# diver-j/melgan-multi

Hardware: NVIDIA H100
Metric: generator_fwd_audio_frames_per_sec (higher is better)
Workload: dtype f32 in/out; products as 3 split-bf16 wgmma passes with fp32 accumulation (fp32-equivalent, ~1e-5)

## Files before the change

melgan_multi_b200/csrc/mg_api.cu:

```cuda
#include <new>
#include <stdlib.h>
#include <string.h>

#include "mg_common.cuh"

namespace mg {


static int *status_ptr(void *workspace, int B, int T) {
    return reinterpret_cast<int *>(reinterpret_cast<float *>(workspace) + ws_offset(6, (size_t)B, (size_t)T));
}

static int run_generator(const float *packed, const float *mel, float *audio, const RunTable &batch, float *ws, cudaStream_t s,
                         cudaEvent_t *ev, const float *mel_host = nullptr, float *audio_host = nullptr) {
    int *st = status_ptr(ws, batch.items(), batch.stride);
    MG_CUDA_TRY(cudaMemsetAsync(st, 0, sizeof(int), s));
    return launch_generator_tc(packed, mel, audio, batch, ws, st, s, ev, mel_host, audio_host);
}

static int check_shape(const char *fn, int B, int T) {
    if (B < 1 || T < 1) return set_error(MG_ERR_INVALID_ARGUMENT, "%s: need B >= 1 and T >= 1 (got B=%d, T=%d)", fn, B, T);
    if ((long long)B * T > (1ll << 24)) return set_error(MG_ERR_INVALID_ARGUMENT, "%s: B*T = %lld too large", fn, (long long)B * T);
    return MG_OK;
}
// ... 126 lines not shown
    int rc = check_shape("mg_gen_stage_output", B, T);
    if (rc) return rc;
    if (which < 0 || which > 3 || !workspace || !out)
        return set_error(MG_ERR_INVALID_ARGUMENT, "mg_gen_stage_output: which must be 0..3 (the last stage is fused with conv_post)");
    if (which > 0 && generator_tc_tail() != 0)
        return set_error(MG_ERR_INVALID_ARGUMENT, "mg_gen_stage_output: ResBlock outputs are not materialised while the next stage's "
                         "ConvT is fused at their kernel's tail; select the unfused chain with mg_gen_set_pipeline(0) first");
    const size_t off = ws_offset(which, B, T), n = ws_offset(which + 1, B, T) - off;
    MG_CUDA_TRY(cudaMemcpyAsync(out, (const float *)workspace + off, n * sizeof(float), cudaMemcpyDeviceToDevice,
                                (cudaStream_t)stream));
    return MG_OK;
}

size_t mg_msd_grouped_backward_workspace_bytes(int layer, int Bt, int Lout) {
    if (layer < 1 || layer > 4 || Bt < 1 || Lout < 1) return 0;
    return grouped_bwd_workspace_bytes(layer, Bt, Lout);
}

int mg_msd_grouped_backward(const void *packed, int scale, int layer, const float *dz, const float *x, float *dx, float *dw,
                            float *db, void *workspace, size_t workspace_bytes, int Bt, int Lin, int Lout, void *stream) {
    if (!packed || !dz || scale < 0 || scale > 2 || layer < 1 || layer > 4 || Bt < 1 || Lin < 1 || Lout < 1)
        return set_error(MG_ERR_INVALID_ARGUMENT, "mg_msd_grouped_backward: bad argument");
    const DLayer d = d_layer(layer);
    if (Lout != (Lin + 2 * d.pad - d.k) / d.stride + 1)
        return set_error(MG_ERR_INVALID_ARGUMENT, "mg_msd_grouped_backward: Lout %d does not follow from Lin %d", Lout, Lin);
    if (dw && (!x || !db || !workspace || workspace_bytes < grouped_bwd_workspace_bytes(layer, Bt, Lout)))
        return set_error(MG_ERR_WORKSPACE_TOO_SMALL, "mg_msd_grouped_backward: dw needs x, db and a workspace of %zu bytes",
                         grouped_bwd_workspace_bytes(layer, Bt, Lout));
    const uint8_t *blob = reinterpret_cast<const uint8_t *>(packed) + (size_t)scale * d_blob_bytes();
    return launch_disc_grouped_backward(blob, layer, dz, x, dx, dw, db, (float *)workspace, Bt, Lin, Lout, (cudaStream_t)stream);
}

int mg_msd_post1_dgrad(const void *packed, int scale, const float *dz, float *dx, int Bt, int L, void *status_word, void *stream) {
    if (!packed || !dz || !dx || dz == dx || !status_word || scale < 0 || scale > 2 || Bt < 1 || L < 1)
        return set_error(MG_ERR_INVALID_ARGUMENT, "mg_msd_post1_dgrad: bad argument");
    const uint8_t *blob = reinterpret_cast<const uint8_t *>(packed) + (size_t)scale * d_blob_bytes();
    return launch_disc_post1_dgrad_tc(dz, dx, blob + d_tcT_start(), reinterpret_cast<const float *>(blob + d_zero_start()), Bt, L,
                                      (int *)status_word, (cudaStream_t)stream);
}

int mg_msd_post1_wgrad(const float *x, const float *dz, float *dw, float *db, int Bt, int L, void *status_word, void *stream) {
    if (!x || !dz || !dw || !db || !status_word || Bt < 1 || L < 1)
        return set_error(MG_ERR_INVALID_ARGUMENT, "mg_msd_post1_wgrad: bad argument");
    return launch_disc_post1_wgrad_tc(x, dz, dw, db, Bt, L, (int *)status_word, (cudaStream_t)stream);
}

size_t mg_msd_edge_backward_workspace_bytes(int layer, int Bt, int L) {
    return (layer == 0 && Bt > 0 && L > 0) ? edge_bwd_workspace_bytes(layer, Bt, L) : 0;
}

int mg_msd_edge_backward(const void *packed, int scale, int layer, const float *dz, const float *x, float *dx, float *dw, float *db,
                         void *workspace, size_t workspace_bytes, int Bt, int L, void *stream) {
    if (!packed || !dz || !x || !dw || !db || scale < 0 || scale > 2 || (layer != 0 && layer != 6) || Bt < 1 || L < 1)
        return set_error(MG_ERR_INVALID_ARGUMENT, "mg_msd_edge_backward: bad argument (layer is 0 = conv_pre or 6 = conv_post2)");
    if (layer == 0 && (!workspace || workspace_bytes < edge_bwd_workspace_bytes(0, Bt, L)))
        return set_error(MG_ERR_WORKSPACE_TOO_SMALL, "mg_msd_edge_backward: conv_pre needs a workspace of %zu bytes",
                         edge_bwd_workspace_bytes(0, Bt, L));
    const uint8_t *blob = reinterpret_cast<const uint8_t *>(packed) + (size_t)scale * d_blob_bytes();
    return launch_disc_edge_backward(blob, layer, dz, x, dx, dw, db, (float *)workspace, Bt, L, (cudaStream_t)stream);
}

size_t mg_msd_scale_backward_workspace_bytes(int Bt, int L0) {
    return (Bt > 0 && L0 > 0) ? disc_scale_backward_workspace_bytes(Bt, L0) : 0;
}

int mg_msd_scale_backward(const void *packed, int scale, const float *x0, const float *const *fmap, const float *const *gfmap,
                          float *gx0, float *const *dw, float *const *db, int *reached, void *workspace, size_t workspace_bytes,
                          int Bt, int L0, void *status_word, void *stream) {
    if (!packed || !x0 || !fmap || !gfmap || !dw || !db || !workspace || !status_word || scale < 0 || scale > 2 || Bt < 1 || L0 < 1)
        return set_error(MG_ERR_INVALID_ARGUMENT, "mg_msd_scale_backward: bad argument");
    for (int l = 0; l < kDiscLayers; ++l)
        if (!fmap[l]) return set_error(MG_ERR_INVALID_ARGUMENT, "mg_msd_scale_backward: fmap[%d] is NULL", l);
    if (Bt > 65535) return set_error(MG_ERR_INVALID_ARGUMENT, "discriminator batch %d exceeds 65535", Bt);
    const uint8_t *blob = reinterpret_cast<const uint8_t *>(packed) + (size_t)scale * d_blob_bytes();
    return launch_disc_scale_backward(blob, x0, fmap, gfmap, gx0, dw, db, reached, workspace, workspace_bytes, Bt, L0,
                                      (int *)status_word, (cudaStream_t)stream);
}

int mg_lrelu_backward(const float *g1, const float *g2, const float *out, float *dz, long long n, void *stream) {
    return launch_lrelu_grad(g1, g2, out, dz, n, (cudaStream_t)stream);
}

int mg_msd_wn_backward(const float *const *v, const float *const *g, const float *const *dw, float *const *dv,
                       float *const *dg, void *stream) {
    if (!v || !g || !dw || !dv || !dg) return set_error(MG_ERR_INVALID_ARGUMENT, "mg_msd_wn_backward: null argument");
    return launch_disc_wn_backward(v, g, dw, dv, dg, (cudaStream_t)stream);
}

int mg_adam_chunk(void) { return 4096; }

int mg_adam_step(float *const *p, const float *const *g, float *const *m, float *const *v, const long long *n,
                 const int *first, int count, int total_ctas, float lr, float beta1, float beta2, float eps,
                 float weight_decay, long long step, void *stream) {
    return launch_adam(p, g, m, v, n, first, count, total_ctas, lr, beta1, beta2, eps, weight_decay, step, (cudaStream_t)stream);
}

size_t mg_loss_workspace_bytes(const long long *n, int count) {
    if (!n || count < 1) return 0;
    return (size_t)loss_num_ctas(n, count) * sizeof(float);
}

int mg_loss_forward(const float *const *a, const float *const *b, const long long *n, const int *mode, int count,
                    float *out, void *workspace, size_t workspace_bytes, void *stream) {
    if (!out || !workspace) return set_error(MG_ERR_INVALID_ARGUMENT, "mg_loss_forward: null argument");
    if (n && count >= 1 && workspace_bytes < mg_loss_workspace_bytes(n, count))
        return set_error(MG_ERR_WORKSPACE_TOO_SMALL, "mg_loss_forward: workspace too small");
    return launch_loss_forward(a, b, n, mode, count, out, (float *)workspace, (cudaStream_t)stream);
}

int mg_loss_backward(const float *const *a, const float *const *b, const long long *n, const int *mode, int count,
                     const float *grad_out, float *const *grad_a, float *const *grad_b, void *stream) {
    if (!grad_out) return set_error(MG_ERR_INVALID_ARGUMENT, "mg_loss_backward: null grad_out");
    return launch_loss_backward(a, b, n, mode, count, grad_out, grad_a, grad_b, (cudaStream_t)stream);
}

int mg_gen_forward_launches(void) { return generator_tc_num_launches(); }

int mg_gen_forward_slices(int B, int T) { return (B >= 1 && T >= 1) ? generator_tc_slices(B, (long long)B * T) : 1; }

int mg_gen_check_status(const void *workspace, int B, int T, void *stream) {
    int rc = check_shape("mg_gen_check_status", B, T);
    if (rc) return rc;
    if (!workspace) return set_error(MG_ERR_INVALID_ARGUMENT, "mg_gen_check_status: null workspace");
    MG_CUDA_TRY(cudaStreamSynchronize((cudaStream_t)stream));
    int st = 0;
    MG_CUDA_TRY(cudaMemcpy(&st, status_ptr(const_cast<void *>(workspace), B, T), sizeof(int), cudaMemcpyDeviceToHost));
    if (st) return set_error(MG_ERR_CUDA, "tensor-core pipeline wait timed out (role code %d)", st);
    return MG_OK;
}

int mg_gen_convt(const void *packed, int stage, const float *x, float *y, int B, int Lin, void *stream) {
    if (!packed || !x || !y || x == y || stage < 0 || stage > 3 || B < 1 || Lin < 1)
        return set_error(MG_ERR_INVALID_ARGUMENT, "mg_gen_convt: bad argument");
    return run_one_kernel("mg_gen_convt", (cudaStream_t)stream, [&](int *st) {
        return launch_convt_tc(x, y, (const float *)packed, stage, RunTable::uniform(B, Lin), st, (cudaStream_t)stream);
    });
}

int mg_gen_conv_pre(const void *packed, const float *mel, float *y, int B, int T, void *stream) {
    if (!packed || !mel || !y || B < 1 || T < 1) return set_error(MG_ERR_INVALID_ARGUMENT, "mg_gen_conv_pre: bad argument");
    return run_one_kernel("mg_gen_conv_pre", (cudaStream_t)stream, [&](int *st) {
        return launch_gen_pre_tc(mel, y, (const float *)packed, RunTable::uniform(B, T), st, (cudaStream_t)stream);
    });
}

int mg_gen_resblock_post(const void *packed, const float *x, float *audio, int B, int L, void *stream) {
    if (!packed || !x || !audio || B < 1 || L < 1) return set_error(MG_ERR_INVALID_ARGUMENT, "mg_gen_resblock_post: bad argument");
    return run_one_kernel("mg_gen_resblock_post", (cudaStream_t)stream, [&](int *st) {
        return launch_resblock_tc(x, audio, (const float *)packed, 4, RunTable::uniform(B, L), st, (cudaStream_t)stream);
    });
}

int mg_gen_resblock_trace(const void *packed, int stage, const float *x, float *y, int B, int L, long long *trace_host) {
    if (!packed || !x || !y || x == y || !trace_host || stage < 0 || stage > 3)
        return set_error(MG_ERR_INVALID_ARGUMENT, "mg_gen_resblock_trace: bad argument");
    int *st = nullptr;
    long long *tr = nullptr;
    MG_CUDA_TRY(cudaMalloc(&st, sizeof(int)));
    MG_CUDA_TRY(cudaMalloc(&tr, 128 * sizeof(long long)));
    cudaMemset(st, 0, sizeof(int));
    cudaMemset(tr, 0, 128 * sizeof(long long));
    int rc = launch_resblock_tc(x, y, (const float *)packed, stage, RunTable::uniform(B, L), st, 0, tr);
    if (rc == MG_OK && cudaDeviceSynchronize() != cudaSuccess) rc = set_error(MG_ERR_CUDA, "mg_gen_resblock_trace: kernel failed");
    if (rc == MG_OK) cudaMemcpy(trace_host, tr, 128 * sizeof(long long), cudaMemcpyDeviceToHost);
    cudaFree(st);
    cudaFree(tr);
    return rc;
}

int mg_gen_resblock(const void *packed, int stage, const float *x, float *y, int B, int L, void *stream) {
    if (!packed || !x || !y || x == y || stage < 0 || stage > 3 || B < 1 || L < 1)
        return set_error(MG_ERR_INVALID_ARGUMENT, "mg_gen_resblock: bad argument");
    return run_one_kernel("mg_gen_resblock", (cudaStream_t)stream, [&](int *st) {
        return launch_resblock_tc(x, y, (const float *)packed, stage, RunTable::uniform(B, L), st, (cudaStream_t)stream);
    });
}

int mg_gen_resup(const void *packed, int stage, const float *x, float *y, int B, int L, void *stream) {
    if (!packed || !x || !y || x == y || stage < 0 || stage > 2 || B < 1 || L < 1)
        return set_error(MG_ERR_INVALID_ARGUMENT, "mg_gen_resup: bad argument");
    return run_one_kernel("mg_gen_resup", (cudaStream_t)stream, [&](int *st) {
        return launch_resblock_tc(x, y, (const float *)packed, 20 + stage, RunTable::uniform(B, L), st, (cudaStream_t)stream);
    });
}

int mg_gen_upres(const void *packed, int stage, const float *x, float *y, int B, int Lin, void *stream) {
    if (!packed || !x || !y || x == y || (stage != 2 && stage != 3) || B < 1 || Lin < 1)
        return set_error(MG_ERR_INVALID_ARGUMENT, "mg_gen_upres: bad argument");
    return run_one_kernel("mg_gen_upres", (cudaStream_t)stream, [&](int *st) {
        return launch_resblock_tc(x, y, (const float *)packed, 10 + stage, RunTable::uniform(B, 2 * Lin), st, (cudaStream_t)stream);
    });
}

int mg_gen_upres_post(const void *packed, const float *x, float *audio, int B, int Lin, void *stream) {
    if (!packed || !x || !audio || (const void *)x == (const void *)audio || B < 1 || Lin < 1)
        return set_error(MG_ERR_INVALID_ARGUMENT, "mg_gen_upres_post: bad argument");
    return run_one_kernel("mg_gen_upres_post", (cudaStream_t)stream, [&](int *st) {
        return launch_resblock_tc(x, audio, (const float *)packed, 14, RunTable::uniform(B, 2 * Lin), st, (cudaStream_t)stream);
    });
}

const char *mg_gen_resblock_config(int code) { return resblock_config_name(code, 0); }


size_t mg_msd_packed_bytes(void) { return msd_packed_bytes(); }

int mg_msd_pack(const float *const *v, const float *const *g, const float *const *bias, void *packed, void *stream) {
    if (!v || !g || !bias || !packed) return set_error(MG_ERR_INVALID_ARGUMENT, "mg_msd_pack: null argument");
    if ((uintptr_t)packed % 256) return set_error(MG_ERR_INVALID_ARGUMENT, "mg_msd_pack: packed must be 256-byte aligned");
    return launch_disc_pack(v, g, bias, packed, (cudaStream_t)stream);
}

int mg_msd_lengths(int L, int *lens) {
    if (L < 1 || !lens) return set_error(MG_ERR_INVALID_ARGUMENT, "mg_msd_lengths: bad argument");
    msd_lengths(L, lens);
    for (int i = 0; i < 21; ++i)
        if (lens[i] < 1) return set_error(MG_ERR_INVALID_ARGUMENT, "mg_msd_lengths: L = %d is too short for the discriminators", L);
    return MG_OK;
}

int mg_msd_forward(const void *packed, const float *y, int Bt, int L, float *const *fmaps, void *status_word, void *stream) {
    if (!packed || !y || !fmaps || !status_word || Bt < 1 || L < 1)
        return set_error(MG_ERR_INVALID_ARGUMENT, "mg_msd_forward: bad argument");
    int lens[21];
    int rc = mg_msd_lengths(L, lens);
    if (rc) return rc;
    for (int i = 0; i < 21; ++i)
        if (!fmaps[i]) return set_error(MG_ERR_INVALID_ARGUMENT, "mg_msd_forward: null feature-map pointer %d", i);
    MG_CUDA_TRY(cudaMemsetAsync(status_word, 0, sizeof(int), (cudaStream_t)stream));
    return launch_msd_forward(packed, y, Bt, L, fmaps, (int *)status_word, (cudaStream_t)stream);
}

size_t mg_disc_packed_bytes(void) { return d_blob_bytes(); }

int mg_disc_pack(const float *const *v, const float *const *g, const float *const *bias, void *packed, void *stream) {
    if (!v || !g || !bias || !packed) return set_error(MG_ERR_INVALID_ARGUMENT, "mg_disc_pack: null argument");
    if ((uintptr_t)packed % 256) return set_error(MG_ERR_INVALID_ARGUMENT, "mg_disc_pack: packed must be 256-byte aligned");
    return launch_disc_pack(v, g, bias, packed, (cudaStream_t)stream, 1);
}

int mg_disc_forward(const void *packed, const float *x, int Bt, int L, float *const *fmaps, void *status_word, void *stream) {
    if (!packed || !x || !fmaps || !status_word || Bt < 1 || L < 1)
        return set_error(MG_ERR_INVALID_ARGUMENT, "mg_disc_forward: bad argument");
    int lens[21];
    msd_lengths(L, lens);
    for (int i = 0; i < 7; ++i) {
        if (lens[i] < 1) return set_error(MG_ERR_INVALID_ARGUMENT, "mg_disc_forward: L = %d is too short", L);
        if (!fmaps[i]) return set_error(MG_ERR_INVALID_ARGUMENT, "mg_disc_forward: null feature-map pointer %d", i);
    }
    MG_CUDA_TRY(cudaMemsetAsync(status_word, 0, sizeof(int), (cudaStream_t)stream));
    return launch_disc_forward(packed, x, Bt, L, fmaps, (int *)status_word, (cudaStream_t)stream);
}

int mg_msd_check_status(const void *status_word, void *stream) {
    if (!status_word) return set_error(MG_ERR_INVALID_ARGUMENT, "mg_msd_check_status: null argument");
    MG_CUDA_TRY(cudaStreamSynchronize((cudaStream_t)stream));
    int st = 0;
    MG_CUDA_TRY(cudaMemcpy(&st, status_word, sizeof(int), cudaMemcpyDeviceToHost));
    if (st) return set_error(MG_ERR_CUDA, "tensor-core pipeline wait timed out (role code %d)", st);
    return MG_OK;
}


size_t mg_mel_tables_bytes(void) { return mel_tables_bytes(); }

int mg_mel_tables_build(int sampling_rate, int n_mels, float fmin, float fmax, int norm, void *tables_host) {
    if (!tables_host) return set_error(MG_ERR_INVALID_ARGUMENT, "mg_mel_tables_build: null buffer");
    return mel_tables_build(sampling_rate, n_mels, fmin, fmax, norm, reinterpret_cast<MelTables *>(tables_host));
}

int mg_mel_frames(int L) { return L < 1 ? 0 : mel_frames(L); }

int mg_mel_spectrogram(const void *tables, const float *audio, float *mel, int B, int L, void *stream) {
    if (!tables || !audio || !mel || B < 1 || L < 1) return set_error(MG_ERR_INVALID_ARGUMENT, "mg_mel_spectrogram: bad argument");
    if ((uintptr_t)tables % 16) return set_error(MG_ERR_INVALID_ARGUMENT, "mg_mel_spectrogram: tables must be 16-byte aligned");
    return launch_mel(tables, audio, mel, B, L, (cudaStream_t)stream);
}


struct mg_gen_engine {
    cudaStream_t stream = nullptr;
    cudaEvent_t ev0 = nullptr, ev1 = nullptr;
    float *packed = nullptr;
    float *raw = nullptr;
    float *mel = nullptr, *audio = nullptr, *ws = nullptr;
    float *pin_in = nullptr, *pin_out = nullptr;
    int *pin_status = nullptr;
    size_t cap_frames = 0;
    bool loaded = false;
    float last_ms = 0.f;
};

static void engine_free_io(mg_gen_engine *e) {
    cudaFree(e->mel); cudaFree(e->audio); cudaFree(e->ws);
    cudaFreeHost(e->pin_in); cudaFreeHost(e->pin_out);
    e->mel = e->audio = e->ws = e->pin_in = e->pin_out = nullptr;
    e->cap_frames = 0;
}

static int engine_reserve(mg_gen_engine *e, size_t frames) {
    if (frames <= e->cap_frames) return MG_OK;
    engine_free_io(e);
    MG_CUDA_TRY(cudaMalloc(&e->mel, frames * kMelBins * sizeof(float)));
    MG_CUDA_TRY(cudaMalloc(&e->audio, frames * 256 * sizeof(float)));
    MG_CUDA_TRY(cudaMalloc(&e->ws, mg_gen_workspace_bytes(1, (int)frames)));
    MG_CUDA_TRY(cudaMallocHost(&e->pin_in, frames * kMelBins * sizeof(float)));
    MG_CUDA_TRY(cudaMallocHost(&e->pin_out, frames * 256 * sizeof(float)));
// ... 102 lines not shown
```

melgan_multi_b200/csrc/mg_res_tc.cu:

```cuda
#include <stdlib.h>
#include <string.h>

#include "mg_common.cuh"
#include "mg_tc.cuh"

namespace mg {
using namespace tc;

template <int C_, int NRB_, int RPW_, int NCP_, int NSTAGE_, bool POST_ = false, bool UPF_ = false, int UPT_ = 0, int CS_ = 1>
struct RbCfg {
    static constexpr int C = C_, NRB = NRB_, RPW = RPW_, NCP = NCP_, NSTAGE = NSTAGE_, UPT = UPT_, CS = CS_;
    static constexpr bool POST = POST_;
    static constexpr bool UPF = UPF_;
    static constexpr int P = 64 * NRB;
    static constexpr int NWG = NRB / RPW * NCP;
    static constexpr int NCONS = 128 * NWG;
    static constexpr int NT = NCONS + 32;
    static constexpr int NCW = C / NCP;
    static constexpr int SLACK = 16;
    static constexpr int HALO = 16 + (POST ? 3 : 0);
    static constexpr int HL = HALO + (UPT_ ? 1 : 0);
    static constexpr int ROWS = P + 2 * SLACK;
    static constexpr int XPITCH = ROWS * 16;
    static constexpr int KP = C / 8;
    static constexpr int XBYTES = KP * XPITCH;
    static constexpr int KC = tc_kc(C);
    static constexpr int CHUNK = tc_chunk_bytes(C);
    static constexpr int HALF = CHUNK / 2;
    static constexpr int NCHUNK = tc_chunks_per_conv(C);
    static constexpr int KSL = C / KC;
    static constexpr int TNG = UPT == 8 ? 32 : C / 2, TN = (UPT ? UPT : 1) * TNG, TNCG = (C / 2) / TNG;
    static constexpr int TSLOT = UPT == 8 ? 16384 : 128 * UPT * TNG, TNSLOT = UPT ? TNCG * (C / 16) * (UPT == 8 ? 2 : 1) : 0;
    static_assert(UPT == 0 || ((UPT == 2 || UPT == 8) && TN == C && TSLOT <= CHUNK && !POST_ && !UPF_), "tail ConvT shape");
    static_assert(UPT != 8 || NCW == 128, "stride-8 tail: each column part stores four phases of a channel as one float4");
    static constexpr int UROWS = P / 2 + 2, UPITCH = UROWS * 16, NPB = NRB / 2, UKSL = 2 * C / KC, NUPCH = UPF ? 4 * UKSL : 0;
    static constexpr int SPITCH = P + 4;
    static_assert(!UPF || (NCP == 1 && NPB <= NWG && 2 * KP * UPITCH <= XBYTES && C * SPITCH * 4 <= 2 * XBYTES),
                  "fused ConvT must fit the X region");
    static_assert(!POST || (C == 32 && NCP == 1), "conv_post fusion is for the 32-channel stage");
    static constexpr int PVB = CS * P - HALO - HL, XCH = 9;
    static_assert(CS == 1 || ((CS == 2 || CS == 4) && !POST_ && !UPF_ && UPT_ == 0 && XCH <= SLACK && 2 * XCH <= P),
                  "clusters are for the plain ResBlock");
    static constexpr int SMEM_BYTES = 2 * XBYTES + NSTAGE * CHUNK + 2 * C * 4 + (2 * NSTAGE + (CS > 1 ? 2 : 0) + 1) * 8;
    static_assert(SMEM_BYTES + 1024 <= 227 * 1024, "shared memory budget");
    static_assert(XPITCH / 16 < 16384, "LBO field");
    static_assert(NRB % RPW == 0 && C % NCP == 0 && NCW % 32 == 0, "warpgroup split");
};

template <int RPW, int R>
__device__ __forceinline__ void acc_fence2(float (&a)[RPW][R]) {
#pragma unroll
    for (int r = 0; r < RPW; ++r) acc_fence<R>(a[r]);
}

template <class Cfg>
__global__ void __launch_bounds__(Cfg::NT, 1)
resblock_tc_kernel(const float *__restrict__ x, float *__restrict__ y, const float *__restrict__ packed, int stage,
                   const __grid_constant__ RunTable clusters, int *__restrict__ status, long long *__restrict__ trace) {
    constexpr int C = Cfg::C, P = Cfg::P, SLACK = Cfg::SLACK, HALO = Cfg::HALO, HL = Cfg::HL;
    constexpr int XPITCH = Cfg::XPITCH, XBYTES = Cfg::XBYTES, KC = Cfg::KC, CHUNK = Cfg::CHUNK, NSTAGE = Cfg::NSTAGE;
    constexpr int NCONS = Cfg::NCONS, NCP = Cfg::NCP, NCW = Cfg::NCW, RPW = Cfg::RPW, KSL = Cfg::KSL, NA = NCW / 2;
    constexpr int CS = Cfg::CS, XCH = Cfg::XCH;
    extern __shared__ __align__(1024) uint8_t smem[];
    uint8_t *Xh = smem, *Xl = smem + XBYTES, *ring = smem + 2 * XBYTES;
    float *pend = reinterpret_cast<float *>(ring + NSTAGE * CHUNK);
    float *b1s = pend + C;
    uint64_t *full = reinterpret_cast<uint64_t *>(b1s + C);
    uint64_t *empty = full + NSTAGE;
    uint64_t *hfull = empty + NSTAGE, *hfree = hfull + 1;
    int *item_len = reinterpret_cast<int *>(empty + NSTAGE + (CS > 1 ? 2 : 0));

    const int tid = threadIdx.x, warp = tid >> 5, lane = tid & 31;
    const int crank = blockIdx.x % CS;
    const RunPos cp = clusters.find(blockIdx.x / CS);
    const int clus = cp.unit, Ls = clusters.stride;
    auto item = [&]() { return *reinterpret_cast<volatile int *>(&item_len[0]); };
    auto len = [&]() { return *reinterpret_cast<volatile int *>(&item_len[1]); };
    const int oc = clus == 0 ? 0 : (CS * P - HALO) + (clus - 1) * Cfg::PVB - HL;
    const int o = oc + crank * P;
    const int p_lo = (clus == 0 || crank > 0) ? 0 : HL, p_hi = (crank < CS - 1 || oc + CS * P >= cp.len) ? P : P - HALO;
    const bool interior = (o >= 0 && o + P <= cp.len);
    const int l0 = 5 + 6 * stage;
    const uint8_t *tc_base = reinterpret_cast<const uint8_t *>(packed) + tc_region_start();

    if (tid == 0) {
        item_len[0] = cp.item;
        item_len[1] = cp.len;
        for (int s = 0; s < NSTAGE; ++s) {
            mbar_init(&full[s], 1);
            mbar_init(&empty[s], Cfg::NWG * CS);
        }
        if constexpr (CS > 1) {
            mbar_init(hfull, 1);
            mbar_init(hfree, (crank > 0) + (crank < CS - 1));
        }
        fence_mbar_init();
    }
    for (int i = Cfg::UPF ? 1 << 30 : tid; i < 2 * Cfg::KP * 2 * SLACK; i += Cfg::NT) {
        const int r = i % (2 * SLACK), kp = (i / (2 * SLACK)) % Cfg::KP, hl = i / (2 * SLACK * Cfg::KP);
        const int row = r < SLACK ? r : P + r;
        *reinterpret_cast<uint4 *>((hl ? Xl : Xh) + kp * XPITCH + row * 16) = make_uint4(0, 0, 0, 0);
    }
    for (int i = tid; i < C; i += Cfg::NT) pend[i] = 0.f;
    fence_proxy_async();
    __syncthreads();
    if constexpr (CS > 1) cluster_sync();
    const bool tr = trace && blockIdx.x == (gridDim.x > 1 ? 1u : 0u) && tid == 0;
#define MG_TR(slot) do { if (tr) trace[slot] = clock64(); } while (0)

    if (warp == NCONS / 32) {
        if (lane == 0) {
            int s = 0, ph = 0, j = 0;
            bool ok = true;
            auto put = [&](const uint8_t *src, uint32_t bytes) {
                if (!ok || !mbar_wait(&empty[s], ph ^ 1)) { ok = false; return; }
                mbar_arrive_expect_tx(&full[s], bytes);
                if constexpr (CS == 1) bulk_g2s(ring + s * CHUNK, src, bytes, &full[s]);
                else if (j % CS == crank) bulk_g2s_multicast(ring + s * CHUNK, src, bytes, &full[s], (1 << CS) - 1);
                ++j;
                if (++s == NSTAGE) { s = 0; ph ^= 1; }
            };
            if constexpr (Cfg::UPF) {
                const uint8_t *src = tc_base + tc_upf_offset(stage);
                for (int i = 0; i < Cfg::NUPCH; ++i) put(src + (size_t)i * CHUNK, CHUNK);
            }
            for (int conv = 0; conv < 6; ++conv) {
                const uint8_t *src = tc_base + tc_res_offset(l0 + (conv >> 1) + 3 * (conv & 1));
                for (int i = 0; i < Cfg::NCHUNK; ++i) put(src + (size_t)i * CHUNK, CHUNK);
            }
            if constexpr (Cfg::UPT != 0) {
                const uint8_t *src = tc_base + tc_up_offset(stage + 1);
                for (int i = 0; i < Cfg::TNSLOT; ++i) put(src + (size_t)i * Cfg::TSLOT, Cfg::TSLOT);
            }
            if (!ok) atomicExch(status, 2);
        }
        if constexpr (CS > 1) cluster_sync();
        return;
    }

    const int wgi = warp >> 2, t = tid & 127, q = lane & 3;
    const int rb0 = (wgi / NCP) * RPW, c0 = (wgi % NCP) * NCW;
    const uint64_t adesc_t = desc_template(XPITCH, 128), bdesc_t = desc_template(C * 16, 128);
    const uint32_t xh_addr = smem_u32(Xh), xl_addr = smem_u32(Xl), ring_addr = smem_u32(ring);
    float R[RPW][NA], D[RPW][NA];
    int s = 0, ph = 0, ps = -1;
    bool ok = true;
    auto release = [&](int slot) {
        if constexpr (CS == 1) {
            if (t == 0) mbar_arrive(&empty[slot]);
        } else if (t < CS) {
            mbar_arrive_remote(&empty[slot], t);
        }
    };
    auto chunk_begin = [&]() -> uint32_t {
        ok &= mbar_wait(&full[s], ph);
        acc_fence2(R);
        acc_fence2(D);
        wgmma_fence();
        return ring_addr + s * CHUNK;
    };
    auto chunk_end = [&]() {
        wgmma_commit();
        wgmma_wait<1>();
        if (ps >= 0) release(ps);
        ps = s;
        if (++s == NSTAGE) { s = 0; ph ^= 1; }
    };
    auto drain = [&]() {
        wgmma_wait<0>();
        acc_fence2(R);
        acc_fence2(D);
        if (ps >= 0) release(ps);
        ps = -1;
    };
    auto sync_cons = [&]() { named_bar_sync(1, NCONS); };
    const int nbr = tid == 0 ? crank - 1 : crank + 1;
    const bool tells = tid < 2 && nbr >= 0 && nbr < CS;
    auto x_read = [&]() {
        sync_cons();
        if constexpr (CS > 1)
            if (tells) mbar_arrive_remote(hfree, nbr);
    };
    auto write_x = [&](float (&A)[RPW][NA], const float *bsrc, bool keep_last) {
        const int L = len();
#pragma unroll
        for (int r = 0; r < RPW; ++r)
#pragma unroll
            for (int h = 0; h < 2; ++h) {
                const int p = (rb0 + r) * 64 + frag_row(t, h), tp = o + p;
                const bool inr = interior || (tp >= 0 && tp < L);
                uint8_t *xh = Xh + (c0 >> 3) * XPITCH + (p + SLACK) * 16 + q * 4, *xl = xh + XBYTES;
#pragma unroll
                for (int k = 0; k < NCW / 8; ++k) {
                    const int col = c0 + 8 * k + 2 * q;
                    const float2 bb = *reinterpret_cast<const float2 *>(bsrc + col);
                    const float f0 = inr ? lrelu(A[r][4 * k + 2 * h] + bb.x) : 0.f;
                    const float f1 = inr ? lrelu(A[r][4 * k + 2 * h + 1] + bb.y) : 0.f;
                    uint32_t hi, lo;
                    split2_bf16(f0, f1, hi, lo);
                    *reinterpret_cast<uint32_t *>(xh + k * XPITCH) = hi;
                    *reinterpret_cast<uint32_t *>(xl + k * XPITCH) = lo;
                    if (keep_last && tp == L - 1) *reinterpret_cast<float2 *>(b1s + col) = make_float2(f0, f1);
                }
            }
    };
    bool border = false;
#pragma unroll
    for (int r = 0; r < RPW; ++r)
#pragma unroll
        for (int h = 0; h < 2; ++h) {
            const int p = (rb0 + r) * 64 + frag_row(t, h);
            border |= (crank > 0 && p < XCH) || (crank < CS - 1 && p >= P - XCH);
        }
    constexpr int NXC = 2 * Cfg::KP;
    constexpr uint32_t XCB = XCH * 16;
    constexpr int NW = NCONS / 32;
    auto send_halo = [&]() {
        for (int i = warp + NW * lane; i < 2 * NXC; i += NCONS) {
            const int side = i / NXC, nb = side ? crank + 1 : crank - 1;
            if (nb < 0 || nb >= CS) continue;
            const uint32_t panel = xh_addr + (i % NXC) * XPITCH;
            const int src = side ? P - XCH : 0, dst = side ? -XCH : P;
            bulk_s2s_cluster(mapa(panel + (SLACK + dst) * 16, nb), panel + (SLACK + src) * 16, XCB, mapa(smem_u32(hfull), nb));
        }
    };
    int hand = 0;
    auto hand_off = [&](float (&A)[RPW][NA], const float *bsrc, bool keep_last) {
        if constexpr (CS > 1) {
            if (border && hand > 0) {
                MG_TR(100 + 2 * hand);
                ok &= mbar_wait(hfree, (hand - 1) & 1);
                MG_TR(101 + 2 * hand);
            }
            if (tid == 0) mbar_arrive_expect_tx(hfull, ((crank > 0) + (crank < CS - 1)) * NXC * XCB);
        }
        write_x(A, bsrc, keep_last);
        fence_proxy_async();
        sync_cons();
        if constexpr (CS > 1) send_halo();
        ++hand;
    };
    auto conv_mma = [&](float (&A)[RPW][NA], int dil, bool fresh, int conv) {
        if constexpr (CS > 1) {
            MG_TR(88 + 2 * conv);
            ok &= mbar_wait(hfull, conv & 1);
            MG_TR(89 + 2 * conv);
        }
        MG_TR(64 + 3 * conv);
#pragma unroll 1
        for (int ch = 0; ch < Cfg::NCHUNK; ++ch) {
            const int tap = ch / KSL, ks = ch % KSL;
            const uint64_t bbase = desc_at(bdesc_t, chunk_begin() + c0 * 16);
            if (ch == 0) MG_TR(65 + 3 * conv);
            const uint32_t arow = (SLACK + rb0 * 64 + (tap - 1) * dil) * 16 + ks * (KC / 8) * XPITCH;
#pragma unroll
            for (int pass = 0; pass < 3; ++pass)
#pragma unroll
                for (int k16 = 0; k16 < KC / 16; ++k16) {
                    const uint64_t bdesc = bbase + (uint64_t)(((pass == 2 ? Cfg::HALF : 0) + 2 * k16 * (C * 16)) >> 4);
                    const uint64_t adesc = desc_at(adesc_t, (pass == 1 ? xl_addr : xh_addr) + arow + 2 * k16 * XPITCH);
#pragma unroll
                    for (int r = 0; r < RPW; ++r)
                        wgmma_bf16<NCW>(A[r], adesc + (uint64_t)(r * 64), bdesc, !(fresh && ch == 0 && pass == 0 && k16 == 0));
                }
            chunk_end();
        }
        MG_TR(66 + 3 * conv);
        drain();
    };

    pdl_wait();
    MG_TR(0);
    if constexpr (Cfg::UPF) {
        constexpr int UROWS = Cfg::UROWS, UPITCH = Cfg::UPITCH, SPITCH = Cfg::SPITCH, UKSL = Cfg::UKSL;
        const int b = item(), L = len();
        const int Lin = L >> 1, Lins = Ls >> 1, s0 = (o >> 1) - 1;
#pragma unroll 1
        for (int idx = tid; idx < UROWS * 2 * Cfg::KP; idx += NCONS) {
            const int i = idx % UROWS, kp = idx / UROWS, sp = s0 + i;
            const bool inr = (sp >= 0 && sp < Lin);
            const float *xp = x + ((size_t)b * 2 * C + 8 * kp) * Lins + (inr ? sp : 0);
            float f[8];
#pragma unroll
            for (int j = 0; j < 8; ++j) f[j] = inr ? lrelu(__ldg(xp + (size_t)j * Lins)) : 0.f;
            uint32_t h[4], l[4];
#pragma unroll
            for (int e = 0; e < 4; ++e) split2_bf16(f[2 * e], f[2 * e + 1], h[e], l[e]);
            *reinterpret_cast<uint4 *>(Xh + kp * UPITCH + i * 16) = make_uint4(h[0], h[1], h[2], h[3]);
            *reinterpret_cast<uint4 *>(Xl + kp * UPITCH + i * 16) = make_uint4(l[0], l[1], l[2], l[3]);
        }
        fence_proxy_async();
        sync_cons();
        const uint64_t udesc_t = desc_template(UPITCH, 128);
        const bool mine = wgi < Cfg::NPB;
        const int pb = wgi % Cfg::NPB;
        auto upf_tap = [&](float (&A)[RPW][NA], int k) {
            const int rowoff = (k == 0) ? 2 : (k == 3) ? 0 : 1;
#pragma unroll 1
            for (int ks = 0; ks < UKSL; ++ks) {
                const uint64_t bbase = desc_at(bdesc_t, chunk_begin());
                const uint32_t arow = (rowoff + pb * 64) * 16 + ks * (KC / 8) * UPITCH;
#pragma unroll
                for (int pass = 0; pass < 3; ++pass)
#pragma unroll
                    for (int k16 = 0; k16 < KC / 16; ++k16) {
                        const uint64_t bdesc = bbase + (uint64_t)(((pass == 2 ? Cfg::HALF : 0) + 2 * k16 * (C * 16)) >> 4);
                        const uint64_t adesc = desc_at(udesc_t, (pass == 1 ? xl_addr : xh_addr) + arow + 2 * k16 * UPITCH);
                        wgmma_bf16<NCW>(A[0], adesc, bdesc, !(k < 2 && ks == 0 && pass == 0 && k16 == 0));
                    }
                chunk_end();
            }
        };
        upf_tap(D, 0);
        upf_tap(R, 1);
        upf_tap(D, 2);
        upf_tap(R, 3);
        drain();
        sync_cons();
        float *stg = reinterpret_cast<float *>(Xh);
        const float *ubias = packed + bias_offset(1 + stage);
        if (mine) {
#pragma unroll
            for (int h = 0; h < 2; ++h) {
                const int m = wgi * 64 + frag_row(t, h);
#pragma unroll
                for (int j = 0; j < NA; ++j) {
                    const int col = frag_col(q, (j & ~3) | (j & 1));
                    if ((j & 2) == 2 * h) {
                        const float bj = __ldg(ubias + col);
                        *reinterpret_cast<float2 *>(stg + (size_t)col * SPITCH + 2 * m) = make_float2(R[0][j] + bj, D[0][j] + bj);
                    }
                }
            }
        }
        sync_cons();
#pragma unroll
        for (int r = 0; r < RPW; ++r)
#pragma unroll
            for (int j = 0; j < NA; ++j) {
                const int p = (rb0 + r) * 64 + frag_row(t, (j >> 1) & 1);
                R[r][j] = stg[(size_t)frag_col(q, (j & ~3) | (j & 1)) * SPITCH + p];
            }
        sync_cons();
        for (int i = tid; i < 2 * Cfg::KP * 2 * SLACK; i += NCONS) {
            const int r = i % (2 * SLACK), kp = (i / (2 * SLACK)) % Cfg::KP, hl = i / (2 * SLACK * Cfg::KP);
            const int row = r < SLACK ? r : P + r;
            *reinterpret_cast<uint4 *>((hl ? Xl : Xh) + kp * XPITCH + row * 16) = make_uint4(0, 0, 0, 0);
        }
    } else {
        const int b = item(), L = len();
#pragma unroll
        for (int r = 0; r < RPW; ++r)
#pragma unroll
            for (int h = 0; h < 2; ++h) {
                const int p = (rb0 + r) * 64 + frag_row(t, h), tp = o + p;
                const bool inr = (tp >= 0 && tp < L);
                const float *xp = x + (size_t)b * C * Ls + (inr ? tp : 0);
#pragma unroll
                for (int k = 0; k < NCW / 8; ++k)
#pragma unroll
                    for (int e = 0; e < 2; ++e)
                        R[r][4 * k + 2 * h + e] = inr ? __ldg(xp + (size_t)(c0 + frag_col(q, 4 * k + e)) * Ls) : 0.f;
            }
    }
    hand_off(R, pend, false);
    MG_TR(1);

#pragma unroll 1
    for (int pr = 0; pr < 3; ++pr) {
        const float *bias1 = packed + bias_offset(l0 + pr);
        for (int c = tid; c < C; c += NCONS) b1s[c] = __ldg(bias1 + c);
        MG_TR(2 + 6 * pr);
        conv_mma(D, pr == 0 ? 1 : pr == 1 ? 3 : 9, true, 2 * pr);
        MG_TR(3 + 6 * pr);
        x_read();
        hand_off(D, b1s, false);
        MG_TR(4 + 6 * pr);
        const float *bias2 = packed + bias_offset(l0 + 3 + pr);
        for (int c = tid; c < C; c += NCONS) pend[c] += __ldg(bias2 + c);
        MG_TR(5 + 6 * pr);
        conv_mma(R, 1, false, 2 * pr + 1);
        MG_TR(6 + 6 * pr);
        x_read();
        if (pr < 2 || Cfg::UPT != 0) hand_off(R, pend, Cfg::UPT != 0 && pr == 2);
        MG_TR(7 + 6 * pr);
    }

    if constexpr (Cfg::POST) {
        pdl_trigger();
        float *Q = reinterpret_cast<float *>(Xh);
        float *wpost = reinterpret_cast<float *>(Xl);
        for (int i = tid; i < 32 * 8; i += NCONS)
            wpost[i] = (i & 7) < kPostK ? __ldg(packed + weight_offset(29) + (i >> 3) * kPostK + (i & 7)) : 0.f;
        sync_cons();
#pragma unroll
        for (int r = 0; r < RPW; ++r)
#pragma unroll
            for (int h = 0; h < 2; ++h) {
                const int p = (rb0 + r) * 64 + frag_row(t, h), tp = o + p;
                const bool inr = (tp >= 0 && tp < len());
                float qk[kPostK];
#pragma unroll
                for (int k = 0; k < kPostK; ++k) qk[k] = 0.f;
#pragma unroll
                for (int k = 0; k < NCW / 8; ++k)
#pragma unroll
                    for (int e = 0; e < 2; ++e) {
                        const int ci = frag_col(q, 4 * k + e);
                        const float a = inr ? lrelu(R[r][4 * k + 2 * h + e] + pend[ci]) : 0.f;
                        const float4 w0 = *reinterpret_cast<const float4 *>(wpost + ci * 8);
                        const float4 w1 = *reinterpret_cast<const float4 *>(wpost + ci * 8 + 4);
                        qk[0] = fmaf(w0.x, a, qk[0]); qk[1] = fmaf(w0.y, a, qk[1]); qk[2] = fmaf(w0.z, a, qk[2]);
                        qk[3] = fmaf(w0.w, a, qk[3]); qk[4] = fmaf(w1.x, a, qk[4]); qk[5] = fmaf(w1.y, a, qk[5]);
                        qk[6] = fmaf(w1.z, a, qk[6]);
                    }
#pragma unroll
                for (int k = 0; k < kPostK; ++k) {
                    qk[k] += __shfl_xor_sync(0xffffffffu, qk[k], 1);
                    qk[k] += __shfl_xor_sync(0xffffffffu, qk[k], 2);
                }
                if (q == 0) {
#pragma unroll
                    for (int k = 0; k < kPostK; ++k) Q[k * P + p] = qk[k];
                }
            }
        sync_cons();
        const int b = item(), L = len();
        const float bpost = __ldg(packed + bias_offset(29));
#pragma unroll 1
        for (int p = tid; p < P; p += NCONS) {
            const int tp = o + p;
            if (p >= p_lo && p < p_hi && tp < L) {
                float acc = bpost;
#pragma unroll
                for (int k = 0; k < kPostK; ++k) {
                    const int pp = p + k - 3;
                    if (pp >= 0 && pp < P) acc += Q[k * P + pp];
                }
                y[(size_t)b * Ls + tp] = tanhf(acc);
            }
        }
        if (oc + P >= L)
            for (int p = L + tid; p < Ls; p += NCONS) y[(size_t)b * Ls + p] = 0.f;
    } else if constexpr (Cfg::UPT != 0) {
        constexpr int S = Cfg::UPT, TNG = Cfg::TNG, TN = Cfg::TN, PADT = S / 2, COT = C / 2;
        const int b = item(), L = len();
        const int Lout = S * Ls;
        const float *tbias = packed + bias_offset(1 + stage + 1);
        {
            const int pl = L - 1 - o;
            if (pl >= p_lo && pl < p_hi) {
                const float *wf = packed + weight_offset(1 + stage + 1);
                for (int i = tid; i < PADT * COT; i += NCONS) {
                    const int co = i / PADT, j = i - co * PADT;
                    const float *wp = wf + ((size_t)co * S + j) * 2 + 1;
                    float acc0 = 0.f, acc1 = 0.f, acc2 = 0.f, acc3 = 0.f;
#pragma unroll 1
                    for (int cc = 0; cc < C; cc += 32) {
                        float wv[32];
#pragma unroll
                        for (int k = 0; k < 32; ++k) wv[k] = __ldg(wp + (size_t)(cc + k) * COT * S * 2);
#pragma unroll
                        for (int k = 0; k < 32; k += 4) {
                            acc0 = fmaf(b1s[cc + k], wv[k], acc0);
                            acc1 = fmaf(b1s[cc + k + 1], wv[k + 1], acc1);
                            acc2 = fmaf(b1s[cc + k + 2], wv[k + 2], acc2);
                            acc3 = fmaf(b1s[cc + k + 3], wv[k + 3], acc3);
                        }
                    }
                    y[((size_t)b * COT + co) * Lout + (size_t)S * L - PADT + j] = (acc0 + acc1) + (acc2 + acc3) + __ldg(tbias + co);
                }
            }
        }
        const uint64_t tbdesc_t = desc_template(TN * 16, 128);
#pragma unroll 1
        for (int cg = 0; cg < Cfg::TNCG; ++cg) {
#pragma unroll 1
            for (int ch = 0; ch < C / 16; ++ch) {
#pragma unroll 1
                for (int ts = 0; ts < (S == 8 ? 2 : 1); ++ts) {
                    const uint64_t bbase = desc_at(tbdesc_t, chunk_begin() + c0 * 16);
#pragma unroll
                    for (int tp = 0; tp < (S == 8 ? 1 : 2); ++tp) {
                        const int tap = S == 8 ? ts : tp;
#pragma unroll
                        for (int pass = 0; pass < 3; ++pass) {
                            const uint32_t boff = (uint32_t)((((S == 8 ? 0 : tp * 2) + (pass == 2 ? 1 : 0)) * 2) * TN * 16);
                            const uint64_t bdesc = bbase + (uint64_t)(boff >> 4);
                            const uint32_t arow = (uint32_t)((SLACK + rb0 * 64 - tap) * 16 + 2 * ch * XPITCH);
                            const uint64_t adesc = desc_at(adesc_t, (pass == 1 ? xl_addr : xh_addr) + arow);
#pragma unroll
                            for (int r = 0; r < RPW; ++r)
                                wgmma_bf16<NCW>(D[r], adesc + (uint64_t)(r * 64), bdesc, !(ch == 0 && tap == 0 && pass == 0));
                        }
                    }
                    chunk_end();
                }
            }
            drain();
            if (cg == Cfg::TNCG - 1) pdl_trigger();
#pragma unroll
            for (int r = 0; r < RPW; ++r)
#pragma unroll
                for (int h = 0; h < 2; ++h) {
                    const int p = (rb0 + r) * 64 + frag_row(t, h), sg = o + p;
                    const bool own = (p >= p_lo && p < p_hi && sg < L);
                    const bool lo_ok = own && sg >= 1, hi_ok = own;
                    if constexpr (S == 8) {
                        const bool ok8 = c0 == 0 ? lo_ok : hi_ok;
                        float *yb = y + ((size_t)b * COT + cg * TNG) * Lout + (own ? 8 * sg - PADT + (c0 >> 5) : 0);
#pragma unroll
                        for (int c = 0; c < 4; ++c)
#pragma unroll
                            for (int e = 0; e < 2; ++e) {
                                const int co = 8 * c + 2 * q + e;
                                const float bj = __ldg(tbias + cg * TNG + co);
                                if (ok8)
                                    *reinterpret_cast<float4 *>(yb + (size_t)co * Lout) =
                                        make_float4(D[r][4 * c + 2 * h + e] + bj, D[r][4 * (4 + c) + 2 * h + e] + bj,
                                                    D[r][4 * (8 + c) + 2 * h + e] + bj, D[r][4 * (12 + c) + 2 * h + e] + bj);
                            }
                    } else {
                        float *yb = y + (size_t)b * COT * Lout + (own ? 2 * sg - PADT : 0);
#pragma unroll
                        for (int k = 0; k < NCW / 8; ++k)
#pragma unroll
                            for (int e = 0; e < 2; ++e) {
                                const int col = c0 + frag_col(q, 4 * k + e), phi = col / TNG, co = col % TNG;
                                if (phi == 0 ? lo_ok : hi_ok) yb[(size_t)co * Lout + phi] = D[r][4 * k + 2 * h + e] + __ldg(tbias + co);
                            }
                    }
                }
        }
    } else {
        pdl_trigger();
        const int b = item(), L = len();
#pragma unroll
        for (int r = 0; r < RPW; ++r)
#pragma unroll
            for (int h = 0; h < 2; ++h) {
                const int p = (rb0 + r) * 64 + frag_row(t, h), tp = o + p;
                if (p >= p_lo && p < p_hi && tp < L) {
                    float *yp = y + (size_t)b * C * Ls + tp;
#pragma unroll
                    for (int k = 0; k < NCW / 8; ++k)
#pragma unroll
                        for (int e = 0; e < 2; ++e) {
                            const int col = c0 + frag_col(q, 4 * k + e);
                            yp[(size_t)col * Ls] = R[r][4 * k + 2 * h + e] + pend[col];
                        }
                }
            }
    }
    if (!ok && t == 0) atomicExch(status, 3);
    if constexpr (CS > 1) cluster_sync();
    MG_TR(20);
#undef MG_TR
}

template <class Cfg>
static int launch_resblock(const float *x, float *y, const float *packed, int stage, const RunTable &batch, int *status,
                           long long *trace, cudaStream_t s) {
    static bool configured = false;
    if (!configured) {
        MG_CUDA_TRY(cudaFuncSetAttribute(resblock_tc_kernel<Cfg>, cudaFuncAttributeMaxDynamicSharedMemorySize, Cfg::SMEM_BYTES));
        configured = true;
    }
    constexpr int CS = Cfg::CS, PC = CS * Cfg::P, PVB = Cfg::PVB;
    RunTable clusters = batch;
    clusters.set_units([](int L) { return 1 + (L > PC ? (L - PC + PVB - 1) / PVB : 0); });
    const dim3 grid(CS * clusters.first[clusters.n]);
    if (trace && CS > 1) {
        cudaLaunchConfig_t cfg{};
        cfg.gridDim = grid;
        cfg.blockDim = dim3(Cfg::NT);
        cfg.dynamicSmemBytes = Cfg::SMEM_BYTES;
        cudaLaunchAttribute attr;
        attr.id = cudaLaunchAttributeClusterDimension;
        attr.val.clusterDim.x = CS;
        attr.val.clusterDim.y = attr.val.clusterDim.z = 1;
        cfg.attrs = &attr;
        cfg.numAttrs = 1;
        int n = 0;
        MG_CUDA_TRY(cudaOccupancyMaxActiveClusters(&n, resblock_tc_kernel<Cfg>, &cfg));
        const long long v = n;
        MG_CUDA_TRY(cudaMemcpy(trace + 127, &v, sizeof(v), cudaMemcpyHostToDevice));
    }
    MG_CUDA_TRY(launch_ex(resblock_tc_kernel<Cfg>, grid, dim3(Cfg::NT), Cfg::SMEM_BYTES, s, true, CS, x, y, packed, stage, clusters,
                          status, trace));
    return MG_OK;
}

template <class Cfg>
static const char *cfg_name() {
    static char buf[96];
    snprintf(buf, sizeof(buf), "resblock_tc_kernel<RbCfg<%d,%d,%d,%d,%d,%d,%d,%d,%d>>", Cfg::C, Cfg::NRB, Cfg::RPW, Cfg::NCP,
             Cfg::NSTAGE, (int)Cfg::POST, (int)Cfg::UPF, Cfg::UPT, Cfg::CS);
    return buf;
}

using Rb0 = RbCfg<256, 1, 1, 2, 4, false, false, 0, 4>;
using Rb1 = RbCfg<128, 2, 1, 1, 4, false, false, 0, 2>;
using Rb2 = RbCfg<64, 4, 1, 1, 3>;
using Rb3 = RbCfg<32, 8, 2, 1, 4>;
using Rb3Post = RbCfg<32, 8, 2, 1, 4, true>;
using Up2Rb2 = RbCfg<64, 4, 1, 1, 3, false, true>;
using Up3Rb3 = RbCfg<32, 8, 2, 1, 4, false, true>;
using Up3Rb3Post = RbCfg<32, 8, 2, 1, 4, true, true>;
using Rb0Up1 = RbCfg<256, 1, 1, 2, 4, false, false, 8>;
using Rb1Up2 = RbCfg<128, 2, 1, 1, 4, false, false, 2>;
using Rb2Up3 = RbCfg<64, 4, 1, 1, 3, false, false, 2>;

int launch_resblock_tc(const float *x, float *y, const float *packed, int stage, const RunTable &batch, int *status, cudaStream_t s,
                       long long *trace) {
    switch (stage) {
        case 0: return launch_resblock<Rb0>(x, y, packed, 0, batch, status, trace, s);
        case 1: return launch_resblock<Rb1>(x, y, packed, 1, batch, status, trace, s);
        case 2: return launch_resblock<Rb2>(x, y, packed, 2, batch, status, trace, s);
        case 3: return launch_resblock<Rb3>(x, y, packed, 3, batch, status, trace, s);
        case 4: return launch_resblock<Rb3Post>(x, y, packed, 3, batch, status, trace, s);
        case 12: return launch_resblock<Up2Rb2>(x, y, packed, 2, batch, status, trace, s);
        case 13: return launch_resblock<Up3Rb3>(x, y, packed, 3, batch, status, trace, s);
        case 14: return launch_resblock<Up3Rb3Post>(x, y, packed, 3, batch, status, trace, s);
        case 20: return launch_resblock<Rb0Up1>(x, y, packed, 0, batch, status, trace, s);
        case 21: return launch_resblock<Rb1Up2>(x, y, packed, 1, batch, status, trace, s);
        case 22: return launch_resblock<Rb2Up3>(x, y, packed, 2, batch, status, trace, s);
    }
    return set_error(MG_ERR_INVALID_ARGUMENT, "launch_resblock_tc: stage %d", stage);
}

const char *resblock_config_name(int stage, int L) {
    (void)L;
    switch (stage) {
        case 0: return cfg_name<Rb0>();
        case 1: return cfg_name<Rb1>();
        case 2: return cfg_name<Rb2>();
        case 3: return cfg_name<Rb3>();
        case 4: return cfg_name<Rb3Post>();
        case 12: return cfg_name<Up2Rb2>();
        case 13: return cfg_name<Up3Rb3>();
        case 14: return cfg_name<Up3Rb3Post>();
        case 20: return cfg_name<Rb0Up1>();
        case 21: return cfg_name<Rb1Up2>();
        case 22: return cfg_name<Rb2Up3>();
    }
    return "";
}

}
```

Measured before the change: 253.6 million.

## Run two smaller ResBlock CTAs per SM and preload all biases once

Adds an occupancy parameter to the ResBlock config, passed into __launch_bounds__, and reconfigures the 64- and 32-channel stages to use half-sized tiles with two CTAs per SM, plus 2-CTA clusters for the plain blocks. All six conv biases and the running residual-bias sums are preloaded into shared memory at kernel start, replacing the per-pass global bias loads and the in-loop pend accumulation. The aim is to overlap one CTA's memory and barrier stalls with another CTA's MMA work. The cost is more halo recomputation from smaller tiles and tighter register and shared-memory budgets.

```diff
diff --git a/melgan_multi_b200/csrc/mg_api.cu b/melgan_multi_b200/csrc/mg_api.cu
--- a/melgan_multi_b200/csrc/mg_api.cu
+++ b/melgan_multi_b200/csrc/mg_api.cu
@@ -302,7 +302,7 @@
 }
 
 int mg_gen_resblock_trace(const void *packed, int stage, const float *x, float *y, int B, int L, long long *trace_host) {
-    if (!packed || !x || !y || x == y || !trace_host || stage < 0 || stage > 3)
+    if (!packed || !x || !y || x == y || !trace_host || !*resblock_config_name(stage, 0) || B < 1 || L < 1)
         return set_error(MG_ERR_INVALID_ARGUMENT, "mg_gen_resblock_trace: bad argument");
     int *st = nullptr;
     long long *tr = nullptr;
diff --git a/melgan_multi_b200/csrc/mg_res_tc.cu b/melgan_multi_b200/csrc/mg_res_tc.cu
--- a/melgan_multi_b200/csrc/mg_res_tc.cu
+++ b/melgan_multi_b200/csrc/mg_res_tc.cu
@@ -7,9 +7,10 @@
 namespace mg {
 using namespace tc;
 
-template <int C_, int NRB_, int RPW_, int NCP_, int NSTAGE_, bool POST_ = false, bool UPF_ = false, int UPT_ = 0, int CS_ = 1>
+template <int C_, int NRB_, int RPW_, int NCP_, int NSTAGE_, bool POST_ = false, bool UPF_ = false, int UPT_ = 0, int CS_ = 1,
+          int OCC_ = 1>
 struct RbCfg {
-    static constexpr int C = C_, NRB = NRB_, RPW = RPW_, NCP = NCP_, NSTAGE = NSTAGE_, UPT = UPT_, CS = CS_;
+    static constexpr int C = C_, NRB = NRB_, RPW = RPW_, NCP = NCP_, NSTAGE = NSTAGE_, UPT = UPT_, CS = CS_, OCC = OCC_;
     static constexpr bool POST = POST_;
     static constexpr bool UPF = UPF_;
     static constexpr int P = 64 * NRB;
@@ -41,8 +42,10 @@
     static constexpr int PVB = CS * P - HALO - HL, XCH = 9;
     static_assert(CS == 1 || ((CS == 2 || CS == 4) && !POST_ && !UPF_ && UPT_ == 0 && XCH <= SLACK && 2 * XCH <= P),
                   "clusters are for the plain ResBlock");
-    static constexpr int SMEM_BYTES = 2 * XBYTES + NSTAGE * CHUNK + 2 * C * 4 + (2 * NSTAGE + (CS > 1 ? 2 : 0) + 1) * 8;
+    static constexpr int NBIAS = 3 + 4 + 1;
+    static constexpr int SMEM_BYTES = 2 * XBYTES + NSTAGE * CHUNK + NBIAS * C * 4 + (2 * NSTAGE + (CS > 1 ? 2 : 0) + 1) * 8;
     static_assert(SMEM_BYTES + 1024 <= 227 * 1024, "shared memory budget");
+    static_assert(OCC * (SMEM_BYTES + 1024) <= 228 * 1024, "OCC CTAs per SM (1 KB reserved per CTA)");
     static_assert(XPITCH / 16 < 16384, "LBO field");
     static_assert(NRB % RPW == 0 && C % NCP == 0 && NCW % 32 == 0, "warpgroup split");
 };
@@ -54,7 +57,7 @@
 }
 
 template <class Cfg>
-__global__ void __launch_bounds__(Cfg::NT, 1)
+__global__ void __launch_bounds__(Cfg::NT, Cfg::OCC)
 resblock_tc_kernel(const float *__restrict__ x, float *__restrict__ y, const float *__restrict__ packed, int stage,
                    const __grid_constant__ RunTable clusters, int *__restrict__ status, long long *__restrict__ trace) {
     constexpr int C = Cfg::C, P = Cfg::P, SLACK = Cfg::SLACK, HALO = Cfg::HALO, HL = Cfg::HL;
@@ -63,9 +66,10 @@
     constexpr int CS = Cfg::CS, XCH = Cfg::XCH;
     extern __shared__ __align__(1024) uint8_t smem[];
     uint8_t *Xh = smem, *Xl = smem + XBYTES, *ring = smem + 2 * XBYTES;
-    float *pend = reinterpret_cast<float *>(ring + NSTAGE * CHUNK);
-    float *b1s = pend + C;
-    uint64_t *full = reinterpret_cast<uint64_t *>(b1s + C);
+    float *b1s = reinterpret_cast<float *>(ring + NSTAGE * CHUNK);
+    float *pend = b1s + 3 * C;
+    float *park = pend + 4 * C;
+    uint64_t *full = reinterpret_cast<uint64_t *>(park + C);
     uint64_t *empty = full + NSTAGE;
     uint64_t *hfull = empty + NSTAGE, *hfree = hfull + 1;
     int *item_len = reinterpret_cast<int *>(empty + NSTAGE + (CS > 1 ? 2 : 0));
@@ -101,7 +105,16 @@
         const int row = r < SLACK ? r : P + r;
         *reinterpret_cast<uint4 *>((hl ? Xl : Xh) + kp * XPITCH + row * 16) = make_uint4(0, 0, 0, 0);
     }
-    for (int i = tid; i < C; i += Cfg::NT) pend[i] = 0.f;
+    for (int i = tid; i < C; i += Cfg::NT) {
+        float acc = 0.f;
+        pend[i] = acc;
+#pragma unroll
+        for (int pr = 0; pr < 3; ++pr) {
+            b1s[pr * C + i] = __ldg(packed + bias_offset(l0 + pr) + i);
+            acc += __ldg(packed + bias_offset(l0 + 3 + pr) + i);
+            pend[(pr + 1) * C + i] = acc;
+        }
+    }
     fence_proxy_async();
     __syncthreads();
     if constexpr (CS > 1) cluster_sync();
@@ -200,7 +213,7 @@
                     split2_bf16(f0, f1, hi, lo);
                     *reinterpret_cast<uint32_t *>(xh + k * XPITCH) = hi;
                     *reinterpret_cast<uint32_t *>(xl + k * XPITCH) = lo;
-                    if (keep_last && tp == L - 1) *reinterpret_cast<float2 *>(b1s + col) = make_float2(f0, f1);
+                    if (keep_last && tp == L - 1) *reinterpret_cast<float2 *>(park + col) = make_float2(f0, f1);
                 }
             }
     };
@@ -368,21 +381,17 @@
 
 #pragma unroll 1
     for (int pr = 0; pr < 3; ++pr) {
-        const float *bias1 = packed + bias_offset(l0 + pr);
-        for (int c = tid; c < C; c += NCONS) b1s[c] = __ldg(bias1 + c);
         MG_TR(2 + 6 * pr);
         conv_mma(D, pr == 0 ? 1 : pr == 1 ? 3 : 9, true, 2 * pr);
         MG_TR(3 + 6 * pr);
         x_read();
-        hand_off(D, b1s, false);
+        hand_off(D, b1s + pr * C, false);
         MG_TR(4 + 6 * pr);
-        const float *bias2 = packed + bias_offset(l0 + 3 + pr);
-        for (int c = tid; c < C; c += NCONS) pend[c] += __ldg(bias2 + c);
         MG_TR(5 + 6 * pr);
         conv_mma(R, 1, false, 2 * pr + 1);
         MG_TR(6 + 6 * pr);
         x_read();
-        if (pr < 2 || Cfg::UPT != 0) hand_off(R, pend, Cfg::UPT != 0 && pr == 2);
+        if (pr < 2 || Cfg::UPT != 0) hand_off(R, pend + (pr + 1) * C, Cfg::UPT != 0 && pr == 2);
         MG_TR(7 + 6 * pr);
     }
 
@@ -407,7 +416,7 @@
 #pragma unroll
                     for (int e = 0; e < 2; ++e) {
                         const int ci = frag_col(q, 4 * k + e);
-                        const float a = inr ? lrelu(R[r][4 * k + 2 * h + e] + pend[ci]) : 0.f;
+                        const float a = inr ? lrelu(R[r][4 * k + 2 * h + e] + pend[3 * C + ci]) : 0.f;
                         const float4 w0 = *reinterpret_cast<const float4 *>(wpost + ci * 8);
                         const float4 w1 = *reinterpret_cast<const float4 *>(wpost + ci * 8 + 4);
                         qk[0] = fmaf(w0.x, a, qk[0]); qk[1] = fmaf(w0.y, a, qk[1]); qk[2] = fmaf(w0.z, a, qk[2]);
@@ -462,10 +471,10 @@
                         for (int k = 0; k < 32; ++k) wv[k] = __ldg(wp + (size_t)(cc + k) * COT * S * 2);
 #pragma unroll
                         for (int k = 0; k < 32; k += 4) {
-                            acc0 = fmaf(b1s[cc + k], wv[k], acc0);
-                            acc1 = fmaf(b1s[cc + k + 1], wv[k + 1], acc1);
-                            acc2 = fmaf(b1s[cc + k + 2], wv[k + 2], acc2);
-                            acc3 = fmaf(b1s[cc + k + 3], wv[k + 3], acc3);
+                            acc0 = fmaf(park[cc + k], wv[k], acc0);
+                            acc1 = fmaf(park[cc + k + 1], wv[k + 1], acc1);
+                            acc2 = fmaf(park[cc + k + 2], wv[k + 2], acc2);
+                            acc3 = fmaf(park[cc + k + 3], wv[k + 3], acc3);
                         }
                     }
                     y[((size_t)b * COT + co) * Lout + (size_t)S * L - PADT + j] = (acc0 + acc1) + (acc2 + acc3) + __ldg(tbias + co);
@@ -547,7 +556,7 @@
 #pragma unroll
                         for (int e = 0; e < 2; ++e) {
                             const int col = c0 + frag_col(q, 4 * k + e);
-                            yp[(size_t)col * Ls] = R[r][4 * k + 2 * h + e] + pend[col];
+                            yp[(size_t)col * Ls] = R[r][4 * k + 2 * h + e] + pend[3 * C + col];
                         }
                 }
             }
@@ -570,6 +579,12 @@
     RunTable clusters = batch;
     clusters.set_units([](int L) { return 1 + (L > PC ? (L - PC + PVB - 1) / PVB : 0); });
     const dim3 grid(CS * clusters.first[clusters.n]);
+    if (trace) {
+        int n = 0;
+        MG_CUDA_TRY(cudaOccupancyMaxActiveBlocksPerMultiprocessor(&n, resblock_tc_kernel<Cfg>, Cfg::NT, Cfg::SMEM_BYTES));
+        const long long v = n;
+        MG_CUDA_TRY(cudaMemcpy(trace + 126, &v, sizeof(v), cudaMemcpyHostToDevice));
+    }
     if (trace && CS > 1) {
         cudaLaunchConfig_t cfg{};
         cfg.gridDim = grid;
@@ -601,12 +616,12 @@
 
 using Rb0 = RbCfg<256, 1, 1, 2, 4, false, false, 0, 4>;
 using Rb1 = RbCfg<128, 2, 1, 1, 4, false, false, 0, 2>;
-using Rb2 = RbCfg<64, 4, 1, 1, 3>;
-using Rb3 = RbCfg<32, 8, 2, 1, 4>;
-using Rb3Post = RbCfg<32, 8, 2, 1, 4, true>;
+using Rb2 = RbCfg<64, 2, 1, 1, 3, false, false, 0, 2, 2>;
+using Rb3 = RbCfg<32, 4, 2, 1, 4, false, false, 0, 2, 2>;
+using Rb3Post = RbCfg<32, 4, 2, 1, 4, true, false, 0, 1, 2>;
 using Up2Rb2 = RbCfg<64, 4, 1, 1, 3, false, true>;
-using Up3Rb3 = RbCfg<32, 8, 2, 1, 4, false, true>;
-using Up3Rb3Post = RbCfg<32, 8, 2, 1, 4, true, true>;
+using Up3Rb3 = RbCfg<32, 4, 2, 1, 4, false, true, 0, 1, 2>;
+using Up3Rb3Post = RbCfg<32, 4, 2, 1, 4, true, true, 0, 1, 2>;
 using Rb0Up1 = RbCfg<256, 1, 1, 2, 4, false, false, 8>;
 using Rb1Up2 = RbCfg<128, 2, 1, 1, 4, false, false, 2>;
 using Rb2Up3 = RbCfg<64, 4, 1, 1, 3, false, false, 2>;
```

Measured after the change: 254.5 million, median of 6. No clear change (+0.3%).
